# salute-developers/GigaAM

Measured on NVIDIA H100. Metric: utterances/sec (10 s audio, v2_ctc), higher is better.
Workload: dtype f16 tensor-core operands, f32 accumulate/residual/norm/head

## Files before the change

### gigaam_b200/csrc/ptx.cuh

```cuda
#pragma once
#include <cuda.h>
#include <cuda_fp16.h>
#include <cuda_runtime.h>
#include <stdint.h>

namespace gam {
namespace ptx {

__device__ __forceinline__ uint32_t smem_u32(const void* p) {
  return static_cast<uint32_t>(__cvta_generic_to_shared(p));
}

__device__ __forceinline__ uint32_t lane_id() {
  uint32_t l;
  asm volatile("mov.u32 %0, %%laneid;" : "=r"(l));
  return l;
}

__device__ __forceinline__ bool elect_one() {
  uint32_t pred = 0;
  asm volatile(
      "{\n\t"
      ".reg .pred P;\n\t"
      "elect.sync _|P, 0xffffffff;\n\t"
      "selp.u32 %0, 1, 0, P;\n\t"
      "}\n"
      : "=r"(pred));
  return pred != 0;
}

__device__ __forceinline__ void mbar_init(uint64_t* bar, uint32_t count) {
  asm volatile("mbarrier.init.shared::cta.b64 [%0], %1;" ::"r"(smem_u32(bar)), "r"(count));
}
__device__ __forceinline__ void fence_mbar_init() {
  asm volatile("fence.mbarrier_init.release.cluster;" ::: "memory");
}
__device__ __forceinline__ void fence_proxy_async_smem() {
  asm volatile("fence.proxy.async.shared::cta;" ::: "memory");
}
__device__ __forceinline__ void mbar_arrive(uint64_t* bar) {
  asm volatile("mbarrier.arrive.shared::cta.b64 _, [%0];" ::"r"(smem_u32(bar)) : "memory");
}
__device__ __forceinline__ void mbar_arrive_expect_tx(uint64_t* bar, uint32_t bytes) {
  asm volatile("mbarrier.arrive.expect_tx.shared::cta.b64 _, [%0], %1;" ::"r"(smem_u32(bar)),
               "r"(bytes)
               : "memory");
}
__device__ __forceinline__ bool mbar_try_wait(uint64_t* bar, uint32_t parity) {
  uint32_t ok;
  asm volatile(
      "{\n\t"
      ".reg .pred P;\n\t"
      "mbarrier.try_wait.parity.shared::cta.b64 P, [%1], %2;\n\t"
      "selp.u32 %0, 1, 0, P;\n\t"
      "}\n"
      : "=r"(ok)
      : "r"(smem_u32(bar)), "r"(parity)
      : "memory");
  return ok != 0;
}
__device__ __forceinline__ void mbar_wait(uint64_t* bar, uint32_t parity) {
  while (!mbar_try_wait(bar, parity)) {
  }
}

__device__ __forceinline__ void prefetch_tmap(const CUtensorMap* m) {
  asm volatile("prefetch.tensormap [%0];" ::"l"(reinterpret_cast<uint64_t>(m)) : "memory");
}
__device__ __forceinline__ void tma_load_2d(void* smem, const CUtensorMap* m, uint64_t* bar, int c0,
                                            int c1) {
  asm volatile(
      "cp.async.bulk.tensor.2d.shared::cluster.global.mbarrier::complete_tx::bytes [%0], [%1, {%3, "
      "%4}], [%2];" ::"r"(smem_u32(smem)),
      "l"(reinterpret_cast<uint64_t>(m)), "r"(smem_u32(bar)), "r"(c0), "r"(c1)
      : "memory");
}
__device__ __forceinline__ void tma_load_2d_multicast(void* smem, const CUtensorMap* m, uint64_t* bar, int c0, int c1,
                                                      uint16_t cta_mask) {
  asm volatile(
      "cp.async.bulk.tensor.2d.shared::cluster.global.mbarrier::complete_tx::bytes.multicast::cluster [%0], [%1, {%3, "
      "%4}], [%2], %5;" ::"r"(smem_u32(smem)),
      "l"(reinterpret_cast<uint64_t>(m)), "r"(smem_u32(bar)), "r"(c0), "r"(c1), "h"(cta_mask)
      : "memory");
}
__device__ __forceinline__ void tma_load_3d(void* smem, const CUtensorMap* m, uint64_t* bar, int c0, int c1, int c2) {
  asm volatile(
      "cp.async.bulk.tensor.3d.shared::cluster.global.mbarrier::complete_tx::bytes [%0], [%1, {%3, "
      "%4, %5}], [%2];" ::"r"(smem_u32(smem)),
      "l"(reinterpret_cast<uint64_t>(m)), "r"(smem_u32(bar)), "r"(c0), "r"(c1), "r"(c2)
      : "memory");
}

__device__ __forceinline__ void tma_load_4d(void* smem, const CUtensorMap* m, uint64_t* bar, int c0,
                                            int c1, int c2, int c3) {
  asm volatile(
      "cp.async.bulk.tensor.4d.shared::cluster.global.mbarrier::complete_tx::bytes [%0], [%1, {%3, "
      "%4, %5, %6}], [%2];" ::"r"(smem_u32(smem)),
      "l"(reinterpret_cast<uint64_t>(m)), "r"(smem_u32(bar)), "r"(c0), "r"(c1), "r"(c2), "r"(c3)
      : "memory");
}
__device__ __forceinline__ void bulk_load(void* smem, const void* gmem, uint32_t bytes, uint64_t* bar) {
  asm volatile("cp.async.bulk.shared::cluster.global.mbarrier::complete_tx::bytes [%0], [%1], %2, [%3];" ::"r"(smem_u32(smem)),
               "l"(reinterpret_cast<uint64_t>(gmem)), "r"(bytes), "r"(smem_u32(bar))
               : "memory");
}
__device__ __forceinline__ void tma_store_2d(const CUtensorMap* m, const void* smem, int c0, int c1) {
  asm volatile(
      "cp.async.bulk.tensor.2d.global.shared::cta.bulk_group [%0, {%2, %3}], [%1];" ::"l"(
          reinterpret_cast<uint64_t>(m)),
      "r"(smem_u32(smem)), "r"(c0), "r"(c1)
      : "memory");
}
__device__ __forceinline__ void tma_store_commit() {
  asm volatile("cp.async.bulk.commit_group;" ::: "memory");
}
template <int N>
__device__ __forceinline__ void tma_store_wait_read() {
  asm volatile("cp.async.bulk.wait_group.read %0;" ::"n"(N) : "memory");
}
template <int N>
__device__ __forceinline__ void tma_store_wait() {
  asm volatile("cp.async.bulk.wait_group %0;" ::"n"(N) : "memory");
}

template <int N>
__device__ __forceinline__ void named_bar_sync(int id) {
  asm volatile("bar.sync %0, %1;" ::"r"(id), "n"(N) : "memory");
}

template <int kRegs>
__device__ __forceinline__ void setmaxnreg_dec() {
  asm volatile("setmaxnreg.dec.sync.aligned.u32 %0;" ::"n"(kRegs));
}
template <int kRegs>
__device__ __forceinline__ void setmaxnreg_inc() {
  asm volatile("setmaxnreg.inc.sync.aligned.u32 %0;" ::"n"(kRegs));
}

__device__ __forceinline__ uint32_t mapa_u32(uint32_t smem_addr, uint32_t cta) {
  uint32_t r;
  asm volatile("mapa.shared::cluster.u32 %0, %1, %2;" : "=r"(r) : "r"(smem_addr), "r"(cta));
  return r;
}
__device__ __forceinline__ uint32_t cluster_ctarank() {
  uint32_t r;
  asm volatile("mov.u32 %0, %%cluster_ctarank;" : "=r"(r));
  return r;
}
__device__ __forceinline__ void cluster_sync() {
  asm volatile("barrier.cluster.arrive.release.aligned;\n\tbarrier.cluster.wait.acquire.aligned;" ::: "memory");
}
__device__ __forceinline__ float ld_cluster_f32(uint32_t addr) {
  float v;
  asm volatile("ld.shared::cluster.f32 %0, [%1];" : "=f"(v) : "r"(addr) : "memory");
  return v;
}
__device__ __forceinline__ int ld_cluster_s32(uint32_t addr) {
  int v;
  asm volatile("ld.shared::cluster.s32 %0, [%1];" : "=r"(v) : "r"(addr) : "memory");
  return v;
}
__device__ __forceinline__ void mbar_arrive_cluster(uint64_t* bar, uint32_t cta) {
  asm volatile("mbarrier.arrive.shared::cluster.b64 _, [%0];" ::"r"(mapa_u32(smem_u32(bar), cta)) : "memory");
}
__device__ __forceinline__ void st_async_v4(uint32_t remote_addr, uint32_t remote_bar, uint32_t a, uint32_t b, uint32_t c,
                                            uint32_t d) {
  asm volatile("st.async.weak.shared::cluster.mbarrier::complete_tx::bytes.v4.b32 [%0], {%1, %2, %3, %4}, [%5];" ::"r"(remote_addr),
               "r"(a), "r"(b), "r"(c), "r"(d), "r"(remote_bar)
               : "memory");
}
__device__ __forceinline__ uint64_t make_wgmma_desc_sw128(uint32_t smem_addr) {
  uint64_t d = 0;
  d |= static_cast<uint64_t>((smem_addr & 0x3FFFF) >> 4);
  d |= static_cast<uint64_t>(1) << 16;
  d |= static_cast<uint64_t>(1024 >> 4) << 32;
  d |= static_cast<uint64_t>(1) << 62;
  return d;
}
__device__ __forceinline__ void wgmma_fence() { asm volatile("wgmma.fence.sync.aligned;" ::: "memory"); }
__device__ __forceinline__ void wgmma_commit() { asm volatile("wgmma.commit_group.sync.aligned;" ::: "memory"); }
template <int N>
__device__ __forceinline__ void wgmma_wait() {
  asm volatile("wgmma.wait_group.sync.aligned %0;" ::"n"(N) : "memory");
}
__device__ __forceinline__ void wgmma_m64n256k16_f16(float* d, uint64_t desc_a, uint64_t desc_b, uint32_t scale_d) {
  asm volatile(
      "{\n\t"
      ".reg .pred p;\n\t"
      "setp.ne.b32 p, %130, 0;\n\t"
      "wgmma.mma_async.sync.aligned.m64n256k16.f32.f16.f16 "
      "{%0, %1, %2, %3, %4, %5, %6, %7, %8, %9, %10, %11, %12, %13, %14, %15, %16, %17, %18, %19, %20, %21, %22, %23, %24, %25, %26, %27, %28, %29, %30, %31, %32, %33, %34, %35, %36, %37, %38, %39, %40, %41, %42, %43, %44, %45, %46, %47, %48, %49, %50, %51, %52, %53, %54, %55, %56, %57, %58, %59, %60, %61, %62, %63, %64, %65, %66, %67, %68, %69, %70, %71, %72, %73, %74, %75, %76, %77, %78, %79, %80, %81, %82, %83, %84, %85, %86, %87, %88, %89, %90, %91, %92, %93, %94, %95, %96, %97, %98, %99, %100, %101, %102, %103, %104, %105, %106, %107, %108, %109, %110, %111, %112, %113, %114, %115, %116, %117, %118, %119, %120, %121, %122, %123, %124, %125, %126, %127}, "
      "%128, %129, p, 1, 1, 0, 0;\n\t"
      "}\n"
      : "+f"(d[0]), "+f"(d[1]), "+f"(d[2]), "+f"(d[3]), "+f"(d[4]), "+f"(d[5]), "+f"(d[6]), "+f"(d[7]), "+f"(d[8]), "+f"(d[9]), "+f"(d[10]), "+f"(d[11]), "+f"(d[12]), "+f"(d[13]), "+f"(d[14]), "+f"(d[15]), "+f"(d[16]), "+f"(d[17]), "+f"(d[18]), "+f"(d[19]), "+f"(d[20]), "+f"(d[21]), "+f"(d[22]), "+f"(d[23]), "+f"(d[24]), "+f"(d[25]), "+f"(d[26]), "+f"(d[27]), "+f"(d[28]), "+f"(d[29]), "+f"(d[30]), "+f"(d[31]), "+f"(d[32]), "+f"(d[33]), "+f"(d[34]), "+f"(d[35]), "+f"(d[36]), "+f"(d[37]), "+f"(d[38]), "+f"(d[39]), "+f"(d[40]), "+f"(d[41]), "+f"(d[42]), "+f"(d[43]), "+f"(d[44]), "+f"(d[45]), "+f"(d[46]), "+f"(d[47]), "+f"(d[48]), "+f"(d[49]), "+f"(d[50]), "+f"(d[51]), "+f"(d[52]), "+f"(d[53]), "+f"(d[54]), "+f"(d[55]), "+f"(d[56]), "+f"(d[57]), "+f"(d[58]), "+f"(d[59]), "+f"(d[60]), "+f"(d[61]), "+f"(d[62]), "+f"(d[63]), "+f"(d[64]), "+f"(d[65]), "+f"(d[66]), "+f"(d[67]), "+f"(d[68]), "+f"(d[69]), "+f"(d[70]), "+f"(d[71]), "+f"(d[72]), "+f"(d[73]), "+f"(d[74]), "+f"(d[75]), "+f"(d[76]), "+f"(d[77]), "+f"(d[78]), "+f"(d[79]), "+f"(d[80]), "+f"(d[81]), "+f"(d[82]), "+f"(d[83]), "+f"(d[84]), "+f"(d[85]), "+f"(d[86]), "+f"(d[87]), "+f"(d[88]), "+f"(d[89]), "+f"(d[90]), "+f"(d[91]), "+f"(d[92]), "+f"(d[93]), "+f"(d[94]), "+f"(d[95]), "+f"(d[96]), "+f"(d[97]), "+f"(d[98]), "+f"(d[99]), "+f"(d[100]), "+f"(d[101]), "+f"(d[102]), "+f"(d[103]), "+f"(d[104]), "+f"(d[105]), "+f"(d[106]), "+f"(d[107]), "+f"(d[108]), "+f"(d[109]), "+f"(d[110]), "+f"(d[111]), "+f"(d[112]), "+f"(d[113]), "+f"(d[114]), "+f"(d[115]), "+f"(d[116]), "+f"(d[117]), "+f"(d[118]), "+f"(d[119]), "+f"(d[120]), "+f"(d[121]), "+f"(d[122]), "+f"(d[123]), "+f"(d[124]), "+f"(d[125]), "+f"(d[126]), "+f"(d[127])
      : "l"(desc_a), "l"(desc_b), "r"(scale_d));
}

__device__ __forceinline__ void ldsm_x4(uint32_t addr, uint32_t& r0, uint32_t& r1, uint32_t& r2, uint32_t& r3) {
  asm volatile("ldmatrix.sync.aligned.m8n8.x4.shared.b16 {%0, %1, %2, %3}, [%4];"
               : "=r"(r0), "=r"(r1), "=r"(r2), "=r"(r3)
               : "r"(addr));
}
__device__ __forceinline__ void ldsm_x4_t(uint32_t addr, uint32_t& r0, uint32_t& r1, uint32_t& r2, uint32_t& r3) {
  asm volatile("ldmatrix.sync.aligned.m8n8.x4.trans.shared.b16 {%0, %1, %2, %3}, [%4];"
               : "=r"(r0), "=r"(r1), "=r"(r2), "=r"(r3)
               : "r"(addr));
}
__device__ __forceinline__ void mma_16816(float* d, const uint32_t* a, uint32_t b0, uint32_t b1) {
  asm volatile(
      "mma.sync.aligned.m16n8k16.row.col.f32.f16.f16.f32 {%0, %1, %2, %3}, {%4, %5, %6, %7}, {%8, %9}, "
      "{%0, %1, %2, %3};"
      : "+f"(d[0]), "+f"(d[1]), "+f"(d[2]), "+f"(d[3])
      : "r"(a[0]), "r"(a[1]), "r"(a[2]), "r"(a[3]), "r"(b0), "r"(b1));
}
__device__ __forceinline__ uint32_t sw128_off(int row, int col) {
  return static_cast<uint32_t>(row * 128 + ((((col >> 3) ^ row) & 7) << 4));
}
__device__ __forceinline__ uint32_t sw128_off_f32(int row, int col) {
  return static_cast<uint32_t>(row * 128 + ((((col >> 2) ^ row) & 7) << 4));
}

}
}
```

### gigaam_b200/csrc/rowops.cu

```cuda
#include "kernels.h"
#include "launch.cuh"
#include "ptx.cuh"

namespace gam {

namespace {

constexpr int kD = 768;
constexpr int kVec = kD / 128;

__device__ __forceinline__ float warp_sum(float v) {
#pragma unroll
  for (int o = 16; o > 0; o >>= 1) v += __shfl_xor_sync(0xffffffffu, v, o);
  return v;
}

__device__ __forceinline__ void load_row_stats(const float* __restrict__ row, int lane, float4 (&v)[kVec],
                                               float& mean, float& rstd, float eps) {
  const float4* r4 = reinterpret_cast<const float4*>(row);
  float s = 0.f;
#pragma unroll
  for (int i = 0; i < kVec; ++i) {
    v[i] = r4[lane + 32 * i];
    s += (v[i].x + v[i].y) + (v[i].z + v[i].w);
  }
  mean = warp_sum(s) * (1.0f / kD);
  float q = 0.f;
#pragma unroll
  for (int i = 0; i < kVec; ++i) {
    float a = v[i].x - mean, b = v[i].y - mean, c = v[i].z - mean, d = v[i].w - mean;
    q += (a * a + b * b) + (c * c + d * d);
  }
  rstd = rsqrtf(warp_sum(q) * (1.0f / kD) + eps);
}

__device__ __forceinline__ int ln_row(int blk, int w, int rows, int reverse) {
  const int r = blk * 8 + w;
  return r >= rows ? -1 : (reverse ? rows - 1 - r : r);
}
__device__ __forceinline__ int live_rows(const int* rows_dev, int rows_max) {
  return rows_dev != nullptr ? min(max(__ldg(rows_dev), 0), rows_max) : rows_max;
}

__device__ __forceinline__ float4 ln_apply(float4 v, float mean, float rstd, float4 g, float4 b) {
  return make_float4((v.x - mean) * rstd * g.x + b.x, (v.y - mean) * rstd * g.y + b.y,
                     (v.z - mean) * rstd * g.z + b.z, (v.w - mean) * rstd * g.w + b.w);
}

__device__ __forceinline__ uint2 pack4(float4 v) {
  __half2 lo = __floats2half2_rn(v.x, v.y), hi = __floats2half2_rn(v.z, v.w);
  return make_uint2(*reinterpret_cast<uint32_t*>(&lo), *reinterpret_cast<uint32_t*>(&hi));
}

__global__ void __launch_bounds__(256) ln_f16_kernel(const float* __restrict__ x, const float* __restrict__ gamma,
                                                     const float* __restrict__ beta, __half* __restrict__ out,
                                                     int rows_max, const int* __restrict__ rows_dev, int reverse, float eps) {
  const int lane = threadIdx.x & 31;
  const int row = ln_row(blockIdx.x, threadIdx.x >> 5, live_rows(rows_dev, rows_max), reverse);
  if (row < 0) return;
  float4 v[kVec];
  float mean, rstd;
  load_row_stats(x + static_cast<size_t>(row) * kD, lane, v, mean, rstd, eps);
  const float4* g4 = reinterpret_cast<const float4*>(gamma);
  const float4* b4 = reinterpret_cast<const float4*>(beta);
  uint2* o = reinterpret_cast<uint2*>(out + static_cast<size_t>(row) * kD);
#pragma unroll
  for (int i = 0; i < kVec; ++i) o[lane + 32 * i] = pack4(ln_apply(v[i], mean, rstd, g4[lane + 32 * i], b4[lane + 32 * i]));
}

__global__ void __launch_bounds__(256) ln_rope_f16_kernel(const float* __restrict__ x, const float* __restrict__ gamma,
                                                          const float* __restrict__ beta,
                                                          const float* __restrict__ rope_cos,
                                                          const float* __restrict__ rope_sin, __half* __restrict__ out_u,
                                                          __half* __restrict__ out_r, int rows_max,
                                                          const int* __restrict__ rows_dev, const int* __restrict__ row_t,
                                                          int T, int half_dim, int reverse, float eps) {
  __shared__ float srow[8][kD];
  const int lane = threadIdx.x & 31;
  const int w = threadIdx.x >> 5;
  const int row = ln_row(blockIdx.x, w, live_rows(rows_dev, rows_max), reverse);
  if (row < 0) return;
  float4 v[kVec];
  float mean, rstd;
  load_row_stats(x + static_cast<size_t>(row) * kD, lane, v, mean, rstd, eps);
  const float4* g4 = reinterpret_cast<const float4*>(gamma);
  const float4* b4 = reinterpret_cast<const float4*>(beta);
  uint2* ou = reinterpret_cast<uint2*>(out_u + static_cast<size_t>(row) * kD);
  float4* s4 = reinterpret_cast<float4*>(srow[w]);
#pragma unroll
  for (int i = 0; i < kVec; ++i) {
    float4 y = ln_apply(v[i], mean, rstd, g4[lane + 32 * i], b4[lane + 32 * i]);
    ou[lane + 32 * i] = pack4(y);
    s4[lane + 32 * i] = y;
  }
  __syncwarp();
  const int t = row_t != nullptr ? __ldg(row_t + row) : row % T;
  const float* cs = rope_cos + static_cast<size_t>(t) * half_dim;
  const float* sn = rope_sin + static_cast<size_t>(t) * half_dim;
  const int hq = half_dim >> 2;
  uint2* orr = reinterpret_cast<uint2*>(out_r + static_cast<size_t>(row) * kD);
#pragma unroll
  for (int i = 0; i < kVec; ++i) {
    const int f4 = lane + 32 * i;
    const int q = f4 % (2 * hq);
    const bool lo = q < hq;
    const float4 a = s4[f4];
    const float4 pt = s4[lo ? f4 + hq : f4 - hq];
    const float sg = lo ? -1.f : 1.f;
    const float4 c = __ldg(reinterpret_cast<const float4*>(cs) + (lo ? q : q - hq));
    const float4 s = __ldg(reinterpret_cast<const float4*>(sn) + (lo ? q : q - hq));
    orr[f4] = pack4(make_float4(fmaf(sg * pt.x, s.x, a.x * c.x), fmaf(sg * pt.y, s.y, a.y * c.y),
                                fmaf(sg * pt.z, s.z, a.z * c.z), fmaf(sg * pt.w, s.w, a.w * c.w)));
  }
}

__global__ void __launch_bounds__(256) ln_out_ln_kernel(const float* __restrict__ r, const float* __restrict__ g_out,
                                                        const float* __restrict__ b_out, const float* __restrict__ g_next,
                                                        const float* __restrict__ b_next, float* __restrict__ x_out,
                                                        __half* __restrict__ y_out, int rows_max,
                                                        const int* __restrict__ rows_dev, int reverse, float eps) {
  const int lane = threadIdx.x & 31;
  const int row = ln_row(blockIdx.x, threadIdx.x >> 5, live_rows(rows_dev, rows_max), reverse);
  if (row < 0) return;
  float4 v[kVec];
  float mean, rstd;
  load_row_stats(r + static_cast<size_t>(row) * kD, lane, v, mean, rstd, eps);
  const float4* g4 = reinterpret_cast<const float4*>(g_out);
  const float4* b4 = reinterpret_cast<const float4*>(b_out);
  float4* xo = reinterpret_cast<float4*>(x_out + static_cast<size_t>(row) * kD);
  float s = 0.f;
#pragma unroll
  for (int i = 0; i < kVec; ++i) {
    v[i] = ln_apply(v[i], mean, rstd, g4[lane + 32 * i], b4[lane + 32 * i]);
    xo[lane + 32 * i] = v[i];
    s += (v[i].x + v[i].y) + (v[i].z + v[i].w);
  }
  if (y_out == nullptr) return;
  mean = warp_sum(s) * (1.0f / kD);
  float q = 0.f;
#pragma unroll
  for (int i = 0; i < kVec; ++i) {
    float a = v[i].x - mean, b = v[i].y - mean, c = v[i].z - mean, d = v[i].w - mean;
    q += (a * a + b * b) + (c * c + d * d);
  }
  rstd = rsqrtf(warp_sum(q) * (1.0f / kD) + eps);
  const float4* gn = reinterpret_cast<const float4*>(g_next);
  const float4* bn = reinterpret_cast<const float4*>(b_next);
  uint2* yo = reinterpret_cast<uint2*>(y_out + static_cast<size_t>(row) * kD);
#pragma unroll
  for (int i = 0; i < kVec; ++i) yo[lane + 32 * i] = pack4(ln_apply(v[i], mean, rstd, gn[lane + 32 * i], bn[lane + 32 * i]));
}

__global__ void __launch_bounds__(256) unpack_rows_kernel(const float* __restrict__ x, const float* __restrict__ gamma,
                                                          const float* __restrict__ beta, const int* __restrict__ cu,
                                                          const int* __restrict__ plen, float* __restrict__ out, int B, int T,
                                                          int reverse, float eps) {
  const int lane = threadIdx.x & 31;
  const int orow = ln_row(blockIdx.x, threadIdx.x >> 5, B * T, reverse);
  if (orow < 0) return;
  const int b = orow / T, t = orow - b * T;
  float4* o = reinterpret_cast<float4*>(out + static_cast<size_t>(orow) * kD);
  if (t >= min(__ldg(plen + b), T)) {
#pragma unroll
    for (int i = 0; i < kVec; ++i) o[lane + 32 * i] = make_float4(0.f, 0.f, 0.f, 0.f);
    return;
  }
  const float* src = x + (static_cast<size_t>(__ldg(cu + b)) + t) * kD;
  float4 v[kVec];
  if (gamma != nullptr) {
    float mean, rstd;
    load_row_stats(src, lane, v, mean, rstd, eps);
    const float4* g4 = reinterpret_cast<const float4*>(gamma);
    const float4* b4 = reinterpret_cast<const float4*>(beta);
#pragma unroll
    for (int i = 0; i < kVec; ++i) o[lane + 32 * i] = ln_apply(v[i], mean, rstd, g4[lane + 32 * i], b4[lane + 32 * i]);
  } else {
#pragma unroll
    for (int i = 0; i < kVec; ++i) o[lane + 32 * i] = reinterpret_cast<const float4*>(src)[lane + 32 * i];
  }
}

constexpr int kDwTT = 32;
constexpr int kDwCT = 128;
constexpr int kDwPerThread = 8;

template <int KW>
__global__ void __launch_bounds__(256) dwconv_bn_silu_kernel(const __half* __restrict__ g, const float* __restrict__ w,
                                                             const float* __restrict__ bias, const int* __restrict__ len,
                                                             const int* __restrict__ cu, const int* __restrict__ plen,
                                                             __half* __restrict__ out, int T) {
  constexpr int kHalo = (KW - 1) / 2;
  constexpr int kRows = kDwTT + KW - 1;
  __shared__ __align__(16) __half2 tile[kRows][kDwCT / 2];
  const int c0 = blockIdx.x * kDwCT;
  const int t0 = blockIdx.y * kDwTT;
  const int b = blockIdx.z;
  const int L = min(len[b], T);
  const int P = cu != nullptr ? min(__ldg(plen + b), T) : T;
  if (t0 >= P) return;
  const size_t base = cu != nullptr ? static_cast<size_t>(__ldg(cu + b)) : static_cast<size_t>(b) * T;
  const __half* gb = g + base * kD;
  for (int i = threadIdx.x; i < kRows * (kDwCT / 8); i += blockDim.x) {
    const int rr = i / (kDwCT / 8), c8 = i % (kDwCT / 8);
    const int t = t0 + rr - kHalo;
    uint4 v = make_uint4(0u, 0u, 0u, 0u);
    if (t >= 0 && t < L) v = *reinterpret_cast<const uint4*>(gb + static_cast<size_t>(t) * kD + c0 + 8 * c8);
    *reinterpret_cast<uint4*>(&tile[rr][4 * c8]) = v;
  }
  __syncthreads();
  const int cp = threadIdx.x % (kDwCT / 2);
  const int tg = threadIdx.x / (kDwCT / 2);
  const int ch = c0 + 2 * cp;
  const int rbase = tg * kDwPerThread;
  float2 x[kDwPerThread + KW - 1];
#pragma unroll
  for (int j = 0; j < kDwPerThread + KW - 1; ++j) x[j] = __half22float2(tile[rbase + j][cp]);
  float a0[kDwPerThread], a1[kDwPerThread];
  const float2 bb = __ldg(reinterpret_cast<const float2*>(bias + ch));
#pragma unroll
  for (int o = 0; o < kDwPerThread; ++o) { a0[o] = bb.x; a1[o] = bb.y; }
  const float2* wt = reinterpret_cast<const float2*>(w + ch);
#pragma unroll
  for (int k = 0; k < KW; ++k) {
    const float2 wk = __ldg(wt + static_cast<size_t>(k) * (kD / 2));
#pragma unroll
    for (int o = 0; o < kDwPerThread; ++o) {
      a0[o] = fmaf(wk.x, x[o + k].x, a0[o]);
      a1[o] = fmaf(wk.y, x[o + k].y, a1[o]);
    }
  }
  __half* ob = out + base * kD;
#pragma unroll
  for (int o = 0; o < kDwPerThread; ++o) {
    const int t = t0 + rbase + o;
    if (t < P) {
      const float h0 = 0.5f * a0[o], h1 = 0.5f * a1[o];
      float t0v, t1v;
      asm("tanh.approx.f32 %0, %1;" : "=f"(t0v) : "f"(h0));
      asm("tanh.approx.f32 %0, %1;" : "=f"(t1v) : "f"(h1));
      *reinterpret_cast<__half2*>(ob + static_cast<size_t>(t) * kD + ch) = __floats2half2_rn(fmaf(h0, t0v, h0), fmaf(h1, t1v, h1));
    }
  }
}

template <int KW>
__global__ void __launch_bounds__(256) dwconv_ln_silu_kernel(const __half* __restrict__ g, const float* __restrict__ w,
                                                             const float* __restrict__ bias, const float* __restrict__ gamma,
                                                             const float* __restrict__ beta, const int* __restrict__ len,
                                                             const int* __restrict__ cu, const int* __restrict__ row_b,
                                                             const int* __restrict__ row_t, const int* __restrict__ rows_dev,
                                                             __half* __restrict__ out, int T, int rows_max, float eps) {
  constexpr int kHalo = (KW - 1) / 2;
  const int lane = threadIdx.x & 31;
  const int row = blockIdx.x * 8 + (threadIdx.x >> 5);
  if (row >= live_rows(rows_dev, rows_max)) return;
  const int b = cu != nullptr ? __ldg(row_b + row) : row / T;
  const int t = cu != nullptr ? __ldg(row_t + row) : row % T;
  const size_t base = cu != nullptr ? static_cast<size_t>(__ldg(cu + b)) : static_cast<size_t>(b) * T;
  const int L = min(len[b], T);
  float acc[24];
#pragma unroll
  for (int i = 0; i < 24; ++i) acc[i] = __ldg(bias + lane * 24 + i);
  for (int k = 0; k < KW; ++k) {
    const int tt = t + k - kHalo;
    if (tt < 0 || tt >= L) continue;
    const __half2* src = reinterpret_cast<const __half2*>(g + (base + tt) * kD + lane * 24);
#pragma unroll
    for (int i = 0; i < 12; ++i) {
      const float2 x = __half22float2(src[i]);
      const float2 wk = __ldg(reinterpret_cast<const float2*>(w + static_cast<size_t>(k) * kD + lane * 24 + 2 * i));
      acc[2 * i] = fmaf(wk.x, x.x, acc[2 * i]);
      acc[2 * i + 1] = fmaf(wk.y, x.y, acc[2 * i + 1]);
    }
  }
  float s = 0.f;
#pragma unroll
  for (int i = 0; i < 24; ++i) s += acc[i];
  const float mean = warp_sum(s) * (1.0f / kD);
  float q = 0.f;
#pragma unroll
  for (int i = 0; i < 24; ++i) { const float d = acc[i] - mean; q += d * d; }
  const float rstd = rsqrtf(warp_sum(q) * (1.0f / kD) + eps);
  __half2* dst = reinterpret_cast<__half2*>(out + static_cast<size_t>(row) * kD + lane * 24);
#pragma unroll
  for (int i = 0; i < 12; ++i) {
    float y0 = (acc[2 * i] - mean) * rstd * __ldg(gamma + lane * 24 + 2 * i) + __ldg(beta + lane * 24 + 2 * i);
    float y1 = (acc[2 * i + 1] - mean) * rstd * __ldg(gamma + lane * 24 + 2 * i + 1) + __ldg(beta + lane * 24 + 2 * i + 1);
    y0 = y0 / (1.f + __expf(-y0));
    y1 = y1 / (1.f + __expf(-y1));
    dst[i] = __floats2half2_rn(y0, y1);
  }
}

__global__ void __launch_bounds__(1024) pack_plan_kernel(const long long* __restrict__ mel_len, int B, int pad2_minus_k, int max_T0,
                                                         int T1, int T2, int* __restrict__ len0, int* __restrict__ len1,
                                                         int* __restrict__ len2, int* __restrict__ plen, int* __restrict__ run1,
                                                         int* __restrict__ cu, int* __restrict__ rows_dev) {
  __shared__ int warp_tot[32];
  __shared__ int carry_s;
  const int lane = threadIdx.x & 31, w = threadIdx.x >> 5, nw = blockDim.x >> 5;
  if (threadIdx.x == 0) carry_s = 0;
  __syncthreads();
  for (int b0 = 0; b0 < B; b0 += blockDim.x) {
    const int b = b0 + threadIdx.x;
    int pl = 0;
    if (b < B) {
      float l = static_cast<float>(mel_len[b]);
      len0[b] = static_cast<int>(min(mel_len[b], static_cast<long long>(max_T0)));
      l = floorf((l + pad2_minus_k) / 2.0f + 1.0f);
      const int l1 = static_cast<int>(l);
      len1[b] = l1;
      l = floorf((l + pad2_minus_k) / 2.0f + 1.0f);
      const int l2 = static_cast<int>(l);
      len2[b] = l2;
      pl = B > 1 ? min(max(l2, 0), T2) : T2;
      plen[b] = pl;
      run1[b] = B > 1 ? min(T1, 2 * ((pl + 7) / 8 * 8) + 2) : T1;
    }
    int v = pl;
#pragma unroll
    for (int o = 1; o < 32; o <<= 1) {
      const int n = __shfl_up_sync(0xffffffffu, v, o);
      if (lane >= o) v += n;
    }
    if (lane == 31) warp_tot[w] = v;
    __syncthreads();
    if (w == 0) {
      int tv = lane < nw ? warp_tot[lane] : 0;
#pragma unroll
      for (int o = 1; o < 32; o <<= 1) {
        const int n = __shfl_up_sync(0xffffffffu, tv, o);
        if (lane >= o) tv += n;
      }
      warp_tot[lane] = tv;
    }
    __syncthreads();
    const int carry = carry_s;
    const int incl = carry + v + (w > 0 ? warp_tot[w - 1] : 0);
    if (b < B) cu[b] = incl - pl;
    __syncthreads();
    if (threadIdx.x == blockDim.x - 1) carry_s = incl;
    __syncthreads();
  }
  if (threadIdx.x == 0) {
    cu[B] = carry_s;
    rows_dev[0] = carry_s;
  }
}

__global__ void row_map_kernel(const int* __restrict__ cu, const int* __restrict__ plen, int T, int* __restrict__ row_b,
                               int* __restrict__ row_t) {
  const int b = blockIdx.y;
  const int t = blockIdx.x * blockDim.x + threadIdx.x;
  if (t < min(plen[b], T)) {
    const int r = cu[b] + t;
    row_b[r] = b;
    row_t[r] = t;
  }
}

}

void launch_ln_f16(const float* x, const float* g, const float* b, __half* out, int rows, const int* rows_dev, int reverse,
                   cudaStream_t s) {
  launch_k(ln_f16_kernel, dim3((rows + 7) / 8), dim3(256), 0, s, x, g, b, out, rows, rows_dev, reverse, 1e-5f);
}
void launch_ln_rope_f16(const float* x, const float* g, const float* b, const float* rc, const float* rs, __half* out_u,
                        __half* out_r, int rows, const int* rows_dev, const int* row_t, int T, int half_dim, int reverse,
                        cudaStream_t s) {
  launch_k(ln_rope_f16_kernel, dim3((rows + 7) / 8), dim3(256), 0, s, x, g, b, rc, rs, out_u, out_r, rows, rows_dev, row_t, T,
           half_dim, reverse, 1e-5f);
}
void launch_ln_out_ln(const float* r, const float* g_out, const float* b_out, const float* g_next, const float* b_next,
                      float* x_out, __half* y_out, int rows, const int* rows_dev, int reverse, cudaStream_t s) {
  launch_k(ln_out_ln_kernel, dim3((rows + 7) / 8), dim3(256), 0, s, r, g_out, b_out, g_next, b_next, x_out, y_out, rows, rows_dev,
           reverse, 1e-5f);
}
void launch_unpack_rows(const float* x, const float* gamma, const float* beta, const int* cu, const int* plen, float* out, int B,
                        int T, int reverse, cudaStream_t s) {
  launch_k(unpack_rows_kernel, dim3((B * T + 7) / 8), dim3(256), 0, s, x, gamma, beta, cu, plen, out, B, T, reverse, 1e-5f);
}
int launch_dwconv_bn_silu(const __half* g, const float* w, const float* bias, const int* len, const int* cu, const int* plen,
                          __half* out, int B, int T, int kw, cudaStream_t s) {
  dim3 grid(kD / kDwCT, (T + kDwTT - 1) / kDwTT, B);
  if (kw == 31) launch_k(dwconv_bn_silu_kernel<31>, grid, dim3(256), 0, s, g, w, bias, len, cu, plen, out, T);
  else if (kw == 5) launch_k(dwconv_bn_silu_kernel<5>, grid, dim3(256), 0, s, g, w, bias, len, cu, plen, out, T);
  else return -1;
  return 0;
}
int launch_dwconv_ln_silu(const __half* g, const float* w, const float* bias, const float* gamma, const float* beta,
                          const int* len, const int* cu, const int* row_b, const int* row_t, const int* rows_dev, __half* out,
                          int B, int T, int kw, cudaStream_t s) {
  const int rows = B * T;
  if (kw == 5)
    dwconv_ln_silu_kernel<5><<<(rows + 7) / 8, 256, 0, s>>>(g, w, bias, gamma, beta, len, cu, row_b, row_t, rows_dev, out, T, rows, 1e-5f);
  else if (kw == 31)
    dwconv_ln_silu_kernel<31><<<(rows + 7) / 8, 256, 0, s>>>(g, w, bias, gamma, beta, len, cu, row_b, row_t, rows_dev, out, T, rows, 1e-5f);
  else return -1;
  return 0;
}
void launch_pack_plan(const long long* mel_len, int B, int pad2_minus_k, int max_T0, int T1, int T2, int* len0, int* len1,
                      int* len2, int* plen, int* run1, int* cu, int* rows_dev, int* row_b, int* row_t, cudaStream_t s) {
  const int threads = B >= 1024 ? 1024 : ((B + 31) / 32 * 32);
  pack_plan_kernel<<<1, threads, 0, s>>>(mel_len, B, pad2_minus_k, max_T0, T1, T2, len0, len1, len2, plen, run1, cu, rows_dev);
  row_map_kernel<<<dim3((T2 + 255) / 256, B), 256, 0, s>>>(cu, plen, T2, row_b, row_t);
}

}
```

Measured before the change: 2800.

## Restructure depthwise conv as streaming per-channel sliding window with cp.async ring

Rewrites the depthwise conv + BN + SiLU kernel so each thread owns one channel and streams a 128-row time strip through a 3-stage cp.async shared-memory ring. A rotating register accumulator computes each output with KW FMAs per input row. This replaces the old tile, which reloaded the KW-1 halo for every 32-row tile. The change aims to cut redundant halo loads and overlap global loads with compute. In exchange, output stores become scalar half writes, and per-thread register pressure for KW=31 goes up.

```diff
diff --git a/gigaam_b200/csrc/ptx.cuh b/gigaam_b200/csrc/ptx.cuh
--- a/gigaam_b200/csrc/ptx.cuh
+++ b/gigaam_b200/csrc/ptx.cuh
@@ -103,6 +103,18 @@
   asm volatile("cp.async.bulk.shared::cluster.global.mbarrier::complete_tx::bytes [%0], [%1], %2, [%3];" ::"r"(smem_u32(smem)),
                "l"(reinterpret_cast<uint64_t>(gmem)), "r"(bytes), "r"(smem_u32(bar))
                : "memory");
+}
+__device__ __forceinline__ void cp_async_16(void* smem, const void* gmem, bool valid) {
+  asm volatile("cp.async.cg.shared.global [%0], [%1], 16, %2;" ::"r"(smem_u32(smem)), "l"(reinterpret_cast<uint64_t>(gmem)),
+               "r"(valid ? 16 : 0)
+               : "memory");
+}
+__device__ __forceinline__ void cp_async_commit() {
+  asm volatile("cp.async.commit_group;" ::: "memory");
+}
+template <int N>
+__device__ __forceinline__ void cp_async_wait() {
+  asm volatile("cp.async.wait_group %0;" ::"n"(N) : "memory");
 }
 __device__ __forceinline__ void tma_store_2d(const CUtensorMap* m, const void* smem, int c0, int c1) {
   asm volatile(
diff --git a/gigaam_b200/csrc/rowops.cu b/gigaam_b200/csrc/rowops.cu
--- a/gigaam_b200/csrc/rowops.cu
+++ b/gigaam_b200/csrc/rowops.cu
@@ -180,67 +180,96 @@
   }
 }
 
-constexpr int kDwTT = 32;
-constexpr int kDwCT = 128;
-constexpr int kDwPerThread = 8;
+constexpr int kDwCT = 256;
+constexpr int kDwStrip = 128;
+constexpr int kDwStages = 3;
 
 template <int KW>
-__global__ void __launch_bounds__(256) dwconv_bn_silu_kernel(const __half* __restrict__ g, const float* __restrict__ w,
-                                                             const float* __restrict__ bias, const int* __restrict__ len,
-                                                             const int* __restrict__ cu, const int* __restrict__ plen,
-                                                             __half* __restrict__ out, int T) {
+constexpr int dw_chunk_rows() { return (32 / KW) * KW; }
+
+template <int KW, bool kFirst, bool kTail>
+__device__ __forceinline__ void dw_chunk(const __half* rows, int i0, int last, const float (&wk)[KW], float bias,
+                                         float (&acc)[KW], __half*& op) {
+  constexpr int kChunk = dw_chunk_rows<KW>();
+#pragma unroll
+  for (int u = 0; u < kChunk; ++u) {
+    if (kTail && i0 + u > last) break;
+    const float x = __half2float(rows[u * kDwCT]);
+    acc[u % KW] = fmaf(wk[0], x, bias);
+#pragma unroll
+    for (int k = 1; k < KW; ++k)
+      if (!kFirst || k <= u) acc[(u - k + KW) % KW] = fmaf(wk[k], x, acc[(u - k + KW) % KW]);
+    if (!kFirst || u >= KW - 1) {
+      const float h = 0.5f * acc[(u + 1) % KW];
+      float th;
+      asm("tanh.approx.f32 %0, %1;" : "=f"(th) : "f"(h));
+      *op = __float2half_rn(fmaf(h, th, h));
+      op += kD;
+    }
+  }
+}
+
+template <int KW>
+__global__ void __launch_bounds__(kDwCT, 3) dwconv_bn_silu_kernel(const __half* __restrict__ g, const float* __restrict__ w,
+                                                                  const float* __restrict__ bias, const int* __restrict__ len,
+                                                                  const int* __restrict__ cu, const int* __restrict__ plen,
+                                                                  __half* __restrict__ out, int T) {
   constexpr int kHalo = (KW - 1) / 2;
-  constexpr int kRows = kDwTT + KW - 1;
-  __shared__ __align__(16) __half2 tile[kRows][kDwCT / 2];
-  const int c0 = blockIdx.x * kDwCT;
-  const int t0 = blockIdx.y * kDwTT;
+  constexpr int kChunk = dw_chunk_rows<KW>();
+  constexpr int kRowStep = kDwCT / (kDwCT / 8);
+  __shared__ __align__(16) __half ring[kDwStages][kChunk][kDwCT];
+  const int t0 = blockIdx.y * kDwStrip;
   const int b = blockIdx.z;
   const int L = min(len[b], T);
   const int P = cu != nullptr ? min(__ldg(plen + b), T) : T;
   if (t0 >= P) return;
   const size_t base = cu != nullptr ? static_cast<size_t>(__ldg(cu + b)) : static_cast<size_t>(b) * T;
-  const __half* gb = g + base * kD;
-  for (int i = threadIdx.x; i < kRows * (kDwCT / 8); i += blockDim.x) {
-    const int rr = i / (kDwCT / 8), c8 = i % (kDwCT / 8);
-    const int t = t0 + rr - kHalo;
-    uint4 v = make_uint4(0u, 0u, 0u, 0u);
-    if (t >= 0 && t < L) v = *reinterpret_cast<const uint4*>(gb + static_cast<size_t>(t) * kD + c0 + 8 * c8);
-    *reinterpret_cast<uint4*>(&tile[rr][4 * c8]) = v;
-  }
-  __syncthreads();
-  const int cp = threadIdx.x % (kDwCT / 2);
-  const int tg = threadIdx.x / (kDwCT / 2);
-  const int ch = c0 + 2 * cp;
-  const int rbase = tg * kDwPerThread;
-  float2 x[kDwPerThread + KW - 1];
-#pragma unroll
-  for (int j = 0; j < kDwPerThread + KW - 1; ++j) x[j] = __half22float2(tile[rbase + j][cp]);
-  float a0[kDwPerThread], a1[kDwPerThread];
-  const float2 bb = __ldg(reinterpret_cast<const float2*>(bias + ch));
-#pragma unroll
-  for (int o = 0; o < kDwPerThread; ++o) { a0[o] = bb.x; a1[o] = bb.y; }
-  const float2* wt = reinterpret_cast<const float2*>(w + ch);
-#pragma unroll
-  for (int k = 0; k < KW; ++k) {
-    const float2 wk = __ldg(wt + static_cast<size_t>(k) * (kD / 2));
-#pragma unroll
-    for (int o = 0; o < kDwPerThread; ++o) {
-      a0[o] = fmaf(wk.x, x[o + k].x, a0[o]);
-      a1[o] = fmaf(wk.y, x[o + k].y, a1[o]);
-    }
-  }
-  __half* ob = out + base * kD;
-#pragma unroll
-  for (int o = 0; o < kDwPerThread; ++o) {
-    const int t = t0 + rbase + o;
-    if (t < P) {
-      const float h0 = 0.5f * a0[o], h1 = 0.5f * a1[o];
-      float t0v, t1v;
-      asm("tanh.approx.f32 %0, %1;" : "=f"(t0v) : "f"(h0));
-      asm("tanh.approx.f32 %0, %1;" : "=f"(t1v) : "f"(h1));
-      *reinterpret_cast<__half2*>(ob + static_cast<size_t>(t) * kD + ch) = __floats2half2_rn(fmaf(h0, t0v, h0), fmaf(h1, t1v, h1));
-    }
-  }
+  const int last = min(kDwStrip, P - t0) + KW - 2;
+  const int chunks = last / kChunk + 1;
+  __shared__ int s_utt[2];
+  const int t_end = min(L, t0 - kHalo + last + 1);
+  if (threadIdx.x == 0) {
+    s_utt[0] = static_cast<int>(base);
+    s_utt[1] = t_end;
+  }
+  auto load = [&](int q, size_t row0, int tend) {
+    const int prow = threadIdx.x / (kDwCT / 8);
+    const int pcol = 8 * (threadIdx.x % (kDwCT / 8));
+    const __half* src = g + row0 * kD + blockIdx.x * kDwCT + pcol;
+    __half(*dst)[kDwCT] = ring[q % kDwStages];
+#pragma unroll
+    for (int j = 0; j < (kChunk + kRowStep - 1) / kRowStep; ++j) {
+      const int rr = prow + kRowStep * j;
+      if (rr < kChunk) {
+        const int t = t0 - kHalo + q * kChunk + rr;
+        const bool live = t >= 0 && t < tend;
+        ptx::cp_async_16(&dst[rr][pcol], src + static_cast<ptrdiff_t>(live ? t : 0) * kD, live);
+      }
+    }
+  };
+#pragma unroll
+  for (int q = 0; q < kDwStages - 1; ++q) {
+    if (q < chunks) load(q, base, t_end);
+    ptx::cp_async_commit();
+  }
+  auto arrive = [&](int q) -> const __half* {
+    ptx::cp_async_wait<kDwStages - 2>();
+    __syncthreads();
+    if (q + kDwStages - 1 < chunks) load(q + kDwStages - 1, static_cast<size_t>(s_utt[0]), s_utt[1]);
+    ptx::cp_async_commit();
+    return &ring[q % kDwStages][0][threadIdx.x];
+  };
+  const int c = blockIdx.x * kDwCT + threadIdx.x;
+  float wk[KW], acc[KW];
+#pragma unroll
+  for (int k = 0; k < KW; ++k) wk[k] = __ldg(w + k * kD + c);
+  const float bc = __ldg(bias + c);
+  __half* op = out + (base + t0) * kD + c;
+  const __half* rows = arrive(0);
+  if (chunks > 1) dw_chunk<KW, true, false>(rows, 0, last, wk, bc, acc, op);
+  else dw_chunk<KW, true, true>(rows, 0, last, wk, bc, acc, op);
+  for (int q = 1; q < chunks - 1; ++q) dw_chunk<KW, false, false>(arrive(q), q * kChunk, last, wk, bc, acc, op);
+  if (chunks > 1) dw_chunk<KW, false, true>(arrive(chunks - 1), (chunks - 1) * kChunk, last, wk, bc, acc, op);
 }
 
 template <int KW>
@@ -382,9 +411,9 @@
 }
 int launch_dwconv_bn_silu(const __half* g, const float* w, const float* bias, const int* len, const int* cu, const int* plen,
                           __half* out, int B, int T, int kw, cudaStream_t s) {
-  dim3 grid(kD / kDwCT, (T + kDwTT - 1) / kDwTT, B);
-  if (kw == 31) launch_k(dwconv_bn_silu_kernel<31>, grid, dim3(256), 0, s, g, w, bias, len, cu, plen, out, T);
-  else if (kw == 5) launch_k(dwconv_bn_silu_kernel<5>, grid, dim3(256), 0, s, g, w, bias, len, cu, plen, out, T);
+  dim3 grid(kD / kDwCT, (T + kDwStrip - 1) / kDwStrip, B);
+  if (kw == 31) launch_k(dwconv_bn_silu_kernel<31>, grid, dim3(kDwCT), 0, s, g, w, bias, len, cu, plen, out, T);
+  else if (kw == 5) launch_k(dwconv_bn_silu_kernel<5>, grid, dim3(kDwCT), 0, s, g, w, bias, len, cu, plen, out, T);
   else return -1;
   return 0;
 }
```

New measurement: 2813 (median of 6 runs). Within noise of the previous version (+0.5%).
